# latk/hbetune.rs

Measured on AMD Instinct MI355X. Metric: GP fit+predict/sec (n=4096,d=8,f64), higher is better.
Workload: dtype f64; 1 GPU; M: rosenbrock d=8 n=4096 f64, Matern nu=5/2 x constant + white noise; fixed-work fit = 3 L-BFGS runs x 150 lml+gradient evaluations + K^-1, then predict mean+variance at m=1600; evals_per_fit=450, n_not_pd=0, m_candidates=1600, parallelism=replicas x1 (independent fits per GPU, no collective)

## Files before the change

### csrc/hbegp.cpp

```cpp
#include "../include/hbegp.h"

#include <hip/hip_runtime_api.h>

#include <algorithm>
#include <atomic>
#include <queue>
#include <cmath>
#include <cstdarg>
#include <cstdio>
#include <cstdlib>
#include <cstring>
#include <functional>
#include <limits>
#include <memory>
#include <mutex>
#include <numeric>
#include <string>
#include <thread>
#include <type_traits>
#include <vector>

#include "dag_plan.hpp"
#include "engine.hpp"
#include "lbfgsb.hpp"
#include "lbfgs_step.hpp"
#include "lockstep.hpp"


using namespace hbegp;

static thread_local std::string g_last_error = "";
static int fail(int code, const char* fmt, ...) {
  char buf[512];
  va_list ap;
  va_start(ap, fmt);
  vsnprintf(buf, sizeof(buf), fmt, ap);
  va_end(ap);
  g_last_error = buf;
  return code;
}
struct HipError {
// ... 549 lines not shown
  }
  off->assign(nwg + 1, 0);
  items->clear();
  for (int w = 0; w < nwg; ++w) {
    (*off)[w] = (int)items->size();
    items->insert(items->end(), per[w].begin(), per[w].end());
  }
  (*off)[nwg] = (int)items->size();
  *nwg_out = nwg;
  return true;
}

constexpr int DAG_MAX_VARIANTS = 4;
constexpr int DAG_CROWD_LEVELS = 3;
constexpr int DAG_CROWD_BUSY[DAG_CROWD_LEVELS] = {6, 12, 24};
constexpr int MAX_DEVS = 64;
struct DagPlanKey {
  int blocks, bk, small_h, nwg, lauum, rl, rl_group, rl_near, lauum_split, chain32, prog, big128;
  auto tie() const { return std::tie(blocks, bk, small_h, nwg, lauum, rl, rl_group, rl_near, lauum_split, chain32, prog, big128); }
  bool operator<(const DagPlanKey& o) const { return tie() < o.tie(); }
};
static std::atomic<int> g_dev_busy[MAX_DEVS];

template <typename T>
struct LooIn {
  int dev;
  hipStream_t s;
  int n, d, np, nu2;
  const T *X, *y, *alpha, *Xinv, *Kinv;
  const EvalParams* P;
};
template <typename T>
static int loo_tail(const LooIn<T>& in, T* mean, T* var, T* lpd, double* loo, double* grad);

template <typename T>
struct Slot {
  int dev = 0;
// ... 3 lines not shown
  T *W1 = nullptr, *W2 = nullptr, *Kinv[2] = {nullptr, nullptr}, *alpha[2] = {nullptr, nullptr};
  T* W3 = nullptr;
  T *ldiag = nullptr, *wbuf = nullptr;
  double *part_t = nullptr, *part_g = nullptr;
  EvalParams* dP = nullptr;
  EvalOut* dOut = nullptr;
  int* tickets = nullptr;
  unsigned long long* dag_trace = nullptr;
  int* dag_ctrl = nullptr;
  EvalParams* hP = nullptr;
  EvalOut* hOut = nullptr;
  void* small_slab = nullptr;
  size_t small_slab_bytes = 0;
  void* host_slab = nullptr;
  size_t host_slab_bytes = 0;
  hipGraphExec_t graph[DAG_MAX_VARIANTS + 1 + DAG_CROWD_LEVELS][2][4] = {};
  int best_idx = -1;
  double best_lml = -std::numeric_limits<double>::infinity();
  int best_run = 0, best_eval = 0;
  std::vector<double> best_theta;
  std::vector<double> best_params;
  int last_target = 0;
  int dag_variant = 1;
  int dag_part = 0;
  unsigned long long seq = 0;
  bool ctrl_cleared = false;
  bool published = false;
  long long expect_ns[4] = {0, 0, 0, 0};
};

struct ProblemBase {
// ... 19 lines not shown
  bool dag_lauum_ = false;
  bool dag_rl_ = false;
  double dag_gflop_lauum = 0;
  struct DagVariant {
    int nwg = 0;
    std::vector<DagTask*> tasks;
    std::vector<DagTask> host_tasks;
    int nwg_p1 = 0, ntasks_p1 = 0, nwg_kinv = 0, ntasks_kinv = 0;
    std::vector<DagTask*> tasks_p1, tasks_kinv;
    std::vector<DagTask> host_tasks_p1, host_tasks_kinv;
  };
  std::vector<DagVariant> dag_var;
  std::unique_ptr<std::atomic<int>[]> busy_slots_;
  int dag_ntasks = 0, dag_nwg = 0;
  int dag_nvar_ = 1, dag_ncrowd_ = 0;
  unsigned long long dag_wait_ticks_ = 200000000ull;
  size_t dag_ctrl_bytes = 0;
  int dag_ctrl_regions_ = 1;
  double dag_gflop = 0;
  bool adhoc_ = false;
  bool small_ = false;
  bool like_fit_ = false;
  bool lazy_ = false;
  std::function<std::shared_ptr<const DagPlan>(int, bool)> plan_for_;
  bool hostio_ = true;
  bool eval_published() const { return hostio_ && !small_; }
  int leaf_dbg_ = 0;

  struct Pooled { int dev; void* p; size_t bytes; };
  std::vector<Pooled> pooled_;
// ... 141 lines not shown
        if (!why.empty()) throw std::runtime_error("task queue of the factorisation is unsound: " + why);
      }
      if (dag_) {
        dag_ntasks = (int)plan.tasks.size();
        dag_nwg = std::min(dag_nwg, dag_ntasks);
        dag_gflop = plan.gflop;
        dag_gflop_lauum = plan.gflop_lauum;
        dag_ctrl_bytes = (sizeof(int) * (DAG_CTRL_WORDS + plan.totals.size()) + 15) / 16 * 16;
        dag_ctrl_regions_ = (lazy_ && dag_lauum_) ? 2 : 1;
        dag_wait_ticks_ = (unsigned long long)(std::max(2.0, 200.0 * plan.sim_us * 1e-6 * std::max(1, n_slots)) * 1e8);
        busy_slots_.reset(new std::atomic<int>[c->devs.size()]);
        for (size_t di = 0; di < c->devs.size(); ++di) busy_slots_[di].store(0);
        const bool adapt = env_int("HBEGP_DAG_ADAPT", 1) != 0 && forced <= 0;
        dag_nvar_ = nvar;
        dag_ncrowd_ = (adapt && n_slots > 1) ? DAG_CROWD_LEVELS : 0;
        dag_var.assign(nvar + 1 + dag_ncrowd_, DagVariant());
        for (int v = 1; v <= nvar + dag_ncrowd_; ++v) {
          DagVariant& var = dag_var[v];
          std::shared_ptr<const DagPlan> pv = cached;
          var.nwg = dag_nwg;
          if (v != nvar && adapt) {
            const int busy = v < nvar ? v : DAG_CROWD_BUSY[v - nvar - 1];
            var.nwg = std::min(share_of(busy), dag_ntasks);
            if (v > nvar) var.nwg = std::min(var.nwg, dag_nwg);
            pv = plan_for(var.nwg);
            if (pv->tasks.size() != plan.tasks.size()) { pv = cached; var.nwg = dag_nwg; }
          }
          var.host_tasks = pv->tasks;
          var.tasks.assign(c->devs.size(), nullptr);
          for (size_t di = 0; di < c->devs.size(); ++di) {
            HIPCHECK(hipSetDevice(c->devs[di]));
            var.tasks[di] = palloc<DagTask>(c->devs[di], pv->tasks.size());
            HIPCHECK(hipMemcpyAsync(var.tasks[di], var.host_tasks.data(), sizeof(DagTask) * var.host_tasks.size(), hipMemcpyHostToDevice, slots[di][0].stream));
          }
          if (lazy_ && dag_lauum_) {
            const int wg_p1 = lazy_wg(var.nwg, 1), wg_kinv = lazy_wg(var.nwg, 2);
            const std::shared_ptr<const DagPlan> p1 = plan_for_(wg_p1, false);
            const DagPlan kv = dag_plan_kinv_only(*pv);
            if (p1->tasks.empty() || kv.tasks.empty() || p1->totals.size() > plan.totals.size() || kv.totals.size() > plan.totals.size()) {
// ... 59 lines not shown
          HIPCHECK(hipMemcpyAsync(sc.d_items, items.data(), sizeof(unsigned) * items.size(), hipMemcpyHostToDevice, s.stream));
          HIPCHECK(hipStreamSynchronize(s.stream));
        }
        scheds[di].push_back(sc);
      };
      eval_gemms(s, s.Kinv[0], record, [](int) {}, [] {});
    }
  }
  ~Problem() override { release(); }

  void release() {
    for (size_t di = 0; di < slots.size(); ++di) {
      (void)hipSetDevice(ctx->devs[di]);
      for (auto& s : slots[di]) {
        if (s.stream) (void)hipStreamSynchronize(s.stream);
        for (int v = 0; v <= DAG_MAX_VARIANTS + DAG_CROWD_LEVELS; ++v)
          for (int a = 0; a < 2; ++a)
            for (int b = 0; b < 4; ++b)
              if (s.graph[v][a][b]) (void)hipGraphExecDestroy(s.graph[v][a][b]);
        const size_t nnb = sizeof(T) * (size_t)np * np;
        g_pool.put(s.dev, s.W1, nnb); g_pool.put(s.dev, s.W2, nnb); g_pool.put(s.dev, s.W3, nnb);
        for (int b = 0; b < 2; ++b) g_pool.put(s.dev, s.Kinv[b], nnb);
        g_pool.put(s.dev, s.small_slab, s.small_slab_bytes);
        g_host_pool.put(s.host_slab, s.host_slab_bytes);
        g_stream_pool.put(s.dev, s.stream);
      }
    }
    for (const Pooled& q : pooled_) g_pool.put(q.dev, q.p, q.bytes);
    pooled_.clear();
    slots.clear();
    scheds.clear();
// ... 272 lines not shown
    keep = base; keep.mi = keep.nj = q0; keep.c_lower = 1; keep.beta_one = 1;
    GemmOp& rect = g.op[g.nops++];
    rect = base; rect.ci0 = q0; rect.mi = nb - q0; rect.nj = q0; rect.klim = 4;
    GemmOp& tri = g.op[g.nops++];
    tri = base; tri.ci0 = tri.cj0 = q0; tri.mi = tri.nj = nb - q0; tri.c_lower = 1; tri.klim = 4;
    gemm_adhoc<T>(g, info, s.stream);
    CHECK_LAUNCHES();
    HIPCHECK(hipMemcpyAsync(s.hOut, s.dOut, sizeof(EvalOut), hipMemcpyDeviceToHost, s.stream));
    HIPCHECK(hipStreamSynchronize(s.stream));
    s.last_target = 0;
    if (s.hOut->info == 0 && !(s.hOut->done & 1)) throw HipError{hipErrorLaunchFailure, "extend: the evaluation kernels did not run", __LINE__};
    if (s.hOut->info == 0 && !std::isfinite(s.hOut->lml)) return HBEGP_NOT_PD;
    return s.hOut->info != 0 ? HBEGP_NOT_PD : HBEGP_OK;
  }

  int variant_now(size_t di) const {
    if (!dag_ || dag_var.size() < 2) return 1;
    const int nvar = dag_nvar_;
    const int busy = busy_slots_ ? busy_slots_[di].load(std::memory_order_relaxed) : 0;
    if (dag_ncrowd_ > 0) {
      const int dev = ctx->devs[di];
      const int total = dev < MAX_DEVS ? g_dev_busy[dev].load(std::memory_order_relaxed) : 0;
      if (total > std::max(busy, nvar)) {
        int l = 0;
        while (l + 1 < dag_ncrowd_ && DAG_CROWD_BUSY[l] < total) ++l;
        return nvar + 1 + l;
      }
    }
    return busy <= 0 ? nvar : std::min(busy, nvar);
  }
  int run_eval(size_t di, int si, int target, int mode, bool use_graph, double* lml, double* grad) {
    Slot<T>& s = slots[di][si];
    HIPCHECK(hipSetDevice(s.dev));
    static const bool graphs_on = env_int("HBEGP_NO_GRAPH", 0) == 0;
    const bool want_grad = mode == EVAL_FULL || mode == EVAL_GRAD_ONLY;
    if (mode == EVAL_GRAD_ONLY) {
      if (!lazy_ || !eval_published() || !grad) throw std::logic_error("run_eval: the gradient phase needs a lazily evaluated, published problem");
      reinterpret_cast<volatile unsigned long long*>(&s.hOut->seq)[0] = 0;
      std::atomic_thread_fence(std::memory_order_seq_cst);
    } else {
      s.dag_variant = variant_now(di);
      s.hP->seq = ++s.seq;
    }
    const auto t_launch = std::chrono::steady_clock::now();
    if (use_graph && graphs_on) {
      hipGraphExec_t& ge = s.graph[s.dag_variant][target][mode];
      if (!ge) {
        hipGraph_t gr = nullptr;
        HIPCHECK(hipStreamBeginCapture(s.stream, hipStreamCaptureModeThreadLocal));
        try {
          enqueue_eval(s, di, target, mode, nullptr);
        } catch (...) {
          (void)hipStreamEndCapture(s.stream, &gr);
          throw;
        }
        HIPCHECK(hipStreamEndCapture(s.stream, &gr));
// ... 1680 lines not shown
  if (!paths) return fail(HBEGP_EINVAL, "NULL paths handle");
  if (!starts || !lo || !hi || !x_best || !f_best) return fail(HBEGP_EINVAL, "starts/lo/hi/x_best/f_best is NULL");
  if (paths->is_f32 != (sizeof(T) == 4)) return fail(HBEGP_EINVAL, "paths handle holds %s data", paths->is_f32 ? "f32" : "f64");
  const int d = paths->model->d;
  if (d > LBFGS_MAXN) return fail(HBEGP_EINVAL, "d = %d exceeds the optimiser's %d variables", d, LBFGS_MAXN);
  for (int k = 0; k < d; ++k)
    if (!(lo[k] <= hi[k])) return fail(HBEGP_EINVAL, "lo[%d] > hi[%d] (%g > %g)", k, k, lo[k], hi[k]);
  for (size_t r = 0; r < (size_t)paths->S * R; ++r)
    for (int k = 0; k < d; ++k) {
      const double v = (double)starts[r * d + k];
      if (!(v >= lo[k] && v <= hi[k])) return fail(HBEGP_EINVAL, "start %zu lies outside the box (feature %d: %g)", r, k, v);
    }
  return HBEGP_OK;
}

struct LastFitStats { int n_evals, n_not_pd, n_lml_only; };
static thread_local LastFitStats g_last_fit_stats = {0, 0, 0};

static int read_fit_options(const hbegp_fit_options* in, hbegp_fit_options* out) {
  *out = hbegp_fit_options{};
  out->struct_size = sizeof(hbegp_fit_options);
  if (!in) return HBEGP_OK;
  if (in->struct_size < offsetof(hbegp_fit_options, maxeval) + sizeof(int) || in->struct_size > ((size_t)1 << 16))
    return fail(HBEGP_EINVAL, "hbegp_fit_options.struct_size = %zu: set it to sizeof(hbegp_fit_options) (HBEGP_FIT_OPTIONS_INIT)",
                in->struct_size);
  memcpy(out, in, std::min(in->struct_size, sizeof(*out)));
  return HBEGP_OK;
}

template <typename T>
static int do_extend(hbegp_ctx* ctx, const T* X, const T* y, int n, int d, double nu, const double* theta, const double* lo,
                     const double* hi, hbegp_model** model_out);

template <typename T>
static int do_fit(hbegp_ctx* ctx, const T* X, const T* y, int n, int d, double nu, const double* theta0, const double* lo,
                  const double* hi, const double* starts, int n_restarts, const hbegp_fit_options* opt_in,
                  double* theta_best, double* lml_best, hbegp_model** model_out, bool loo = false) {
  hbegp_fit_options opt{};
  g_last_fit_stats = {0, 0, 0};
  if (int e = read_fit_options(opt_in, &opt)) return e;
  if (opt.maxeval <= 0) opt.maxeval = 150;
  const int p = d + 2;
  const int nruns = 1 + std::max(0, n_restarts);
  const int ndev = (int)ctx->devs.size();
  const int max_conc = std::max(1, env_int("HBEGP_MAX_CONCURRENT", 3));
  std::vector<int> runs_on(ndev, 0);
  for (int r = 0; r < nruns; ++r) runs_on[r % ndev]++;
  int n_slots = 1;
  for (int di = 0; di < ndev; ++di) n_slots = std::max(n_slots, std::min(runs_on[di], max_conc));
  constexpr int SMALL_FIT_MAX_RUNS = 64;
  bool small_fit = !loo && round_up(n, NB) == NB && d <= SMALL_EVAL_MAXD && env_int("HBEGP_SMALL", 1) != 0 && env_int("HBEGP_SMALL_FIT", 1) != 0;
  for (int di = 0; di < ndev; ++di) small_fit = small_fit && runs_on[di] <= SMALL_FIT_MAX_RUNS;
  if (small_fit)
    for (int di = 0; di < ndev; ++di) n_slots = std::max(n_slots, runs_on[di]);
  static const int timing = env_int("HBEGP_TIMING", 0);
  const auto tf0 = std::chrono::steady_clock::now();
  SmallArrival arrival;
  if (small_fit) arrival.announce();
  static const int host_serial_max = env_int("HBEGP_SMALL_HOST_SERIAL", 16);
  struct SmallActive {
    bool on = false;
    int enter() { on = true; return g_small_active.fetch_add(1) + 1; }
    ~SmallActive() { if (on) g_small_active.fetch_sub(1); }
  } small_active;
  const bool host_serial = small_fit && small_active.enter() <= host_serial_max;
  std::unique_lock<std::mutex> host_lk(g_small_host_mu, std::defer_lock);
  if (host_serial) host_lk.lock();
  const auto th0 = std::chrono::steady_clock::now();
  double held_ms = 0;
  Problem<T> prob(ctx, X, y, n, d, nu, n_slots, false, true, !loo);
  const auto tf1 = std::chrono::steady_clock::now();
// ... 109 lines not shown
          } else {
            std::this_thread::sleep_for(microseconds(40));
            if (steady_clock::now() - last_query > milliseconds(20)) {
              last_query = steady_clock::now();
              const hipError_t e = hipStreamQuery(batches[di]->stream);
              if (e == hipSuccess) {
                if (*q == 1ull) break;
                throw HipError{hipErrorLaunchFailure, "small fit: the launch is over and a run never reported", __LINE__};
              }
              if (e != hipErrorNotReady) throw HipError{e, "hipStreamQuery (small-fit launch)", __LINE__};
            }
          }
        }
        std::atomic_thread_fence(std::memory_order_acquire);
      };
      for (int r = 0; r < nruns; ++r) wait_run(r, ws[r].di);
      runs_over = true;
      int total_evals = 0, total_not_pd = 0, trace_n = 0;
      for (int r = 0; r < nruns; ++r) {
        RunWs& w = ws[r];
        HIPCHECK(hipSetDevice(ctx->devs[w.di]));
        Slot<T>& s = prob.slots[w.di][w.si];
        hipStream_t st = prob.slots[w.di][0].stream;
        const SmallFitResult hr = hruns[r].res;
        total_evals += hr.n_evals;
        total_not_pd += hr.n_not_pd;
        s.best_idx = hr.best_idx;
        s.best_lml = hr.best_lml;
        s.best_run = r;
        s.best_eval = hr.best_eval;
        s.best_theta.assign(hr.best_theta, hr.best_theta + p);
        s.best_params.assign(hr.best_params, hr.best_params + p);
        s.last_target = hr.best_idx < 0 ? 0 : hr.best_idx;
        if (cap > 0 && trace_n < opt.trace_cap) {
          const int take = std::min(std::min(hr.n_evals, cap), opt.trace_cap - trace_n);
          if (opt.trace_theta) HIPCHECK(hipMemcpyAsync(opt.trace_theta + (size_t)trace_n * p, w.tr_theta, sizeof(double) * (size_t)take * p, hipMemcpyDeviceToHost, st));
          if (opt.trace_lml) HIPCHECK(hipMemcpyAsync(opt.trace_lml + trace_n, w.tr_lml, sizeof(double) * take, hipMemcpyDeviceToHost, st));
          if (opt.trace_grad) HIPCHECK(hipMemcpyAsync(opt.trace_grad + (size_t)trace_n * p, w.tr_grad, sizeof(double) * (size_t)take * p, hipMemcpyDeviceToHost, st));
          HIPCHECK(hipStreamSynchronize(st));
          if (opt.trace_run) for (int e = 0; e < take; ++e) opt.trace_run[trace_n + e] = r;
          trace_n += take;
        }
      }
      if (opt.trace_count) *opt.trace_count = trace_n;
      if (opt.n_evals) *opt.n_evals = total_evals;
      if (opt.n_not_pd) *opt.n_not_pd = total_not_pd;
      g_last_fit_stats = {total_evals, total_not_pd, 0};
      n_evals.store(total_evals);
    } catch (...) {
      for (int di = 0; di < ndev && di < (int)prob.slots.size(); ++di) {
        if (prob.slots[di].empty()) continue;
        (void)hipSetDevice(ctx->devs[di]);
        (void)hipStreamSynchronize(prob.slots[di][0].stream);
      }
      free_all();
      throw;
    }
    free_all();
  } else {
  if (prob.busy_slots_)
    for (int di = 0; di < ndev; ++di) prob.busy_slots_[di].store(std::min(runs_on[di], max_conc));
  auto worker = [&](int di, int si) {
    struct Leave {
      std::atomic<int>* busy;
      std::atomic<int>* dev_busy;
      ~Leave() {
        if (busy) busy->fetch_sub(1);
        if (dev_busy) dev_busy->fetch_sub(1);
      }
    } leave{prob.busy_slots_ ? &prob.busy_slots_[di] : nullptr, ctx->devs[di] < MAX_DEVS ? &g_dev_busy[ctx->devs[di]] : nullptr};
    if (leave.dev_busy) leave.dev_busy->fetch_add(1);
    try {
      HIPCHECK(hipSetDevice(ctx->devs[di]));
      Slot<T>& s = prob.slots[di][si];
      const int nslots_here = std::min(runs_on[di], max_conc);
      int local = 0;
      for (int r = di; r < nruns; r += ndev, ++local) {
        if (local % nslots_here != si) continue;
        std::vector<double> x(p);
        if (r == 0) for (int i = 0; i < p; ++i) x[i] = theta0[i];
        else for (int i = 0; i < p; ++i) x[i] = starts[(size_t)(r - 1) * p + i];
        int eval_idx = 0;
        auto obj = [&](const double* th, double* grad, const LbfgsState* ls) -> double {
          theta_to_params(th, lo, hi, d, s.hP);
          const int target = (s.best_idx < 0) ? 0 : 1 - s.best_idx;
          double lml;
          int st;
          if (ls) {
            st = prob.run_eval((size_t)di, si, target, Problem<T>::EVAL_LML_ONLY, true, &lml, nullptr);
            const bool new_best = st == HBEGP_OK && (s.best_idx < 0 || lml > s.best_lml);
            if (st == HBEGP_OK && (new_best || lbfgs_trial_accepted(*ls, -lml))) {
              st = prob.run_eval((size_t)di, si, target, Problem<T>::EVAL_GRAD_ONLY, true, nullptr, grad);
              if (st != HBEGP_OK) lml = -std::numeric_limits<double>::infinity();
            } else {
              for (int j = 0; j < p; ++j) grad[j] = 0.0;
              n_lml_only.fetch_add(1);
            }
          } else {
            st = prob.run_eval((size_t)di, si, target, !loo, true, &lml, loo ? nullptr : grad);
          }
          if (loo) {
            if (st == HBEGP_OK) st = prob.loo_on_slot((size_t)di, si, &lml, grad);
            else for (int j = 0; j < p; ++j) grad[j] = 0.0;
            if (st != HBEGP_OK && st != HBEGP_NOT_PD) throw std::runtime_error(g_last_error);
          }
          const int my_eval = eval_idx++;
          n_evals.fetch_add(1);
          if (st != HBEGP_OK) n_not_pd.fetch_add(1);
          if (opt.trace_cap > 0) {
            std::lock_guard<std::mutex> lk(trace_mu);
            if (trace_n < opt.trace_cap) {
              const int tI = trace_n++;
              if (opt.trace_theta) memcpy(opt.trace_theta + (size_t)tI * p, th, sizeof(double) * p);
              if (opt.trace_lml) opt.trace_lml[tI] = lml;
              if (opt.trace_grad) memcpy(opt.trace_grad + (size_t)tI * p, grad, sizeof(double) * p);
              if (opt.trace_run) opt.trace_run[tI] = r;
            }
          }
          if (st != HBEGP_OK) return std::numeric_limits<double>::infinity();
          if (s.best_idx < 0 || lml > s.best_lml) {
            s.best_idx = target;
// ... 6 lines not shown
          return -lml;
        };
        LbfgsOptions lo_opt;
        lo_opt.maxeval = opt.maxeval;
        lo_opt.fixed_work = opt.fixed_work != 0;
        if (opt.lbfgs_memory > 0) lo_opt.memory = opt.lbfgs_memory;
        static_assert(MAXP <= LBFGS_MAXN, "the GP's parameters fit the fixed-size optimiser state");
        std::vector<double> g(p);
        std::unique_ptr<LbfgsState> ls(new LbfgsState);
        lbfgs_begin(*ls, x.data(), lnlo.data(), lnhi.data(), p, lo_opt.maxeval, lo_opt.memory, lo_opt.pgtol, lo_opt.ftol, lo_opt.fixed_work);
        for (;;) {
          const bool trial = lazy && lbfgs_is_trial(*ls);
          const double f = obj(lbfgs_request(*ls), g.data(), trial ? ls.get() : nullptr);
          if (!lbfgs_advance(*ls, f, g.data())) break;
        }
      }
    } catch (const HipError& he) {
      hip_fail(he);
      std::lock_guard<std::mutex> lk(err_mu);
      err = g_last_error;
    } catch (const std::exception& e) {
      std::lock_guard<std::mutex> lk(err_mu);
      err = std::string("worker thread: ") + e.what();
    }
  };

  std::vector<std::thread> threads;
  try {
    for (int di = 0; di < ndev; ++di)
      for (int si = 0; si < std::min(runs_on[di], max_conc); ++si) threads.emplace_back(worker, di, si);
// ... 8 lines not shown
    std::stable_sort(order.begin(), order.end(), [&](int a, int b) { return opt.trace_run[a] < opt.trace_run[b]; });
    auto permute = [&](auto* arr, int width) {
      if (!arr) return;
      std::vector<typename std::remove_pointer<decltype(arr)>::type> tmp((size_t)trace_n * width);
      for (int i = 0; i < trace_n; ++i) memcpy(&tmp[(size_t)i * width], arr + (size_t)order[i] * width, sizeof(tmp[0]) * width);
      memcpy(arr, tmp.data(), sizeof(tmp[0]) * tmp.size());
    };
    permute(opt.trace_theta, p);
    permute(opt.trace_lml, 1);
    permute(opt.trace_grad, p);
    permute(opt.trace_run, 1);
  }
  if (opt.trace_count) *opt.trace_count = trace_n;
  if (opt.n_evals) *opt.n_evals = n_evals.load();
  if (opt.n_not_pd) *opt.n_not_pd = n_not_pd.load();
  g_last_fit_stats = {n_evals.load(), n_not_pd.load(), n_lml_only.load()};
  if (!err.empty()) return fail(HBEGP_EHIP, "%s", err.c_str());
  }

  int bdi = -1, bsi = -1;
  for (int di = 0; di < ndev; ++di)
    for (int si = 0; si < (int)prob.slots[di].size(); ++si) {
      const Slot<T>& s = prob.slots[di][si];
      if (s.best_idx < 0) continue;
      bool better = bdi < 0;
      if (!better) {
        const Slot<T>& b = prob.slots[bdi][bsi];
        better = s.best_lml > b.best_lml ||
                 (s.best_lml == b.best_lml && (s.best_run < b.best_run || (s.best_run == b.best_run && s.best_eval < b.best_eval)));
      }
      if (better) { bdi = di; bsi = si; }
    }
  if (bdi < 0) return fail(HBEGP_ALL_FAILED, "every evaluation of the fit failed (kernel matrix not positive definite)");
// ... 1209 lines not shown
void hbegp_model_retain(hbegp_model* model) {
  if (model) model->refs.fetch_add(1);
}
void hbegp_model_release(hbegp_model* model) {
  if (model && model->refs.fetch_sub(1) == 1) delete model;
}

int hbegp_last_fit_stats(hbegp_fit_stats* out) {
  if (!out || out->struct_size < offsetof(hbegp_fit_stats, n_evals) + sizeof(int) || out->struct_size > ((size_t)1 << 16))
    return fail(HBEGP_EINVAL, "hbegp_fit_stats.struct_size: set it to sizeof(hbegp_fit_stats) (HBEGP_FIT_STATS_INIT)");
  hbegp_fit_stats full{};
  full.struct_size = out->struct_size;
  full.n_evals = g_last_fit_stats.n_evals;
  full.n_not_pd = g_last_fit_stats.n_not_pd;
  full.n_lml_only = g_last_fit_stats.n_lml_only;
  memcpy(out, &full, std::min(out->struct_size, sizeof(full)));
  return HBEGP_OK;
}

static int lbfgs_replay_impl(int n, const double* x0, const double* lo, const double* hi, int maxeval, int memory, int fixed_work, int count,
                             const double* f, const double* g, double* requested, int* trial, int* accepted, int* took, int* n_requested) {
  LbfgsOptions o;
  std::unique_ptr<LbfgsState> st(new LbfgsState);
  lbfgs_begin(*st, x0, lo, hi, n, maxeval, memory > 0 ? memory : o.memory, o.pgtol, o.ftol, fixed_work != 0);
  memcpy(requested, lbfgs_request(*st), sizeof(double) * n);
  int produced = 1;
  for (int i = 0; i < count; ++i) {
    if (trial) {
      trial[i] = lbfgs_is_trial(*st) ? 1 : 0;
      accepted[i] = lbfgs_trial_accepted(*st, f[i]) ? 1 : 0;
// ... 8 lines not shown
    }
  }
  *n_requested = produced;
  return HBEGP_OK;
}

int hbegp_debug_lbfgs_decisions(int n, const double* x0, const double* lo, const double* hi, int maxeval, int memory, int fixed_work,
                                int count, const double* f, const double* g, double* requested, int* trial, int* accepted, int* took,
                                int* n_requested) {
  if (n < 1 || n > LBFGS_MAXN || count < 0 || !x0 || !lo || !hi || !requested || !n_requested || !trial || !accepted || !took ||
      (count > 0 && (!f || !g)))
    return fail(HBEGP_EINVAL, "bad argument");
  GUARD_BEGIN
  return lbfgs_replay_impl(n, x0, lo, hi, maxeval, memory, fixed_work, count, f, g, requested, trial, accepted, took, n_requested);
  GUARD_END
}

int hbegp_debug_dag_queues(int nblocks, int bk, int small_h, int nwg, int fine, int big128, int which, int* ntasks, int* tasks, int cap,
                           char* err, int errlen) {
  if (nblocks < 1 || (bk != 16 && bk != 32) || small_h < 0 || nwg < 0 || which < 0 || which > 2 || !ntasks) return fail(HBEGP_EINVAL, "bad argument");
  GUARD_BEGIN
  DagBuilder builder(bk, small_h, nwg, (fine & 1) != 0);
  builder.set_rl_progressive((fine & 16) != 0);
  builder.set_big128(big128 != 0, big128 >= 2);
  builder.set_rl(32, 1, (fine & 32) == 0, true);
  DagPlan plan = builder.build(0, nblocks, which != 1, (fine & 8) != 0);
  if (which == 2) plan = dag_plan_kinv_only(plan);
  const std::string why = plan.tasks.empty() ? std::string("no tasks") : dag_plan_validate(plan, nblocks);
  *ntasks = (int)plan.tasks.size();
  if (tasks)
// ... 73 lines not shown
```

### hbetune_rs_amd/_lib.py

```python
import ctypes as C
import os

import numpy as np

HERE = os.path.dirname(os.path.abspath(__file__))
LIB_PATH = os.environ.get("HBEGP_LIB") or os.path.join(HERE, "libhbegp.so")

OK, NOT_PD, ALL_FAILED = 0, 1, 2
EINVAL, EHIP, ENODEV, ENOMEM = -1, -2, -3, -4
PATHS_MAX_FEATURES, PATHS_MAX_PATHS = 16384, 1024
CEI_MAX_CONSTRAINTS = 8
MES_MAX_SAMPLES = 1024
EHVI_ND_MAX_BOXES = 1048576


class HbegpError(RuntimeError):
    def __init__(self, code, msg):
        super().__init__(f"hbegp error {code}: {msg}")
        self.code = code


class FitOptions(C.Structure):

    _fields_ = [
        ("struct_size", C.c_size_t),
        ("maxeval", C.c_int),
        ("fixed_work", C.c_int),
        ("lbfgs_memory", C.c_int),
# ... 2 lines not shown
        ("trace_lml", C.POINTER(C.c_double)),
        ("trace_grad", C.POINTER(C.c_double)),
        ("trace_run", C.POINTER(C.c_int)),
        ("trace_count", C.POINTER(C.c_int)),
        ("n_evals", C.POINTER(C.c_int)),
        ("n_not_pd", C.POINTER(C.c_int)),
    ]

    def __init__(self, *a, **k):
        super().__init__(*a, **k)
        self.struct_size = C.sizeof(FitOptions)


class FitStats(C.Structure):

    _fields_ = [("struct_size", C.c_size_t), ("n_evals", C.c_int), ("n_not_pd", C.c_int), ("n_lml_only", C.c_int)]

    def __init__(self, *a, **k):
        super().__init__(*a, **k)
        self.struct_size = C.sizeof(FitStats)


OBJECTIVE_FN = C.CFUNCTYPE(C.c_double, C.POINTER(C.c_double), C.POINTER(C.c_double), C.c_void_p)

_dp = C.POINTER(C.c_double)
_fp = C.POINTER(C.c_float)
_ip = C.POINTER(C.c_int)
_vp = C.c_void_p

SIGNATURES = {
    "hbegp_version": (C.c_int, []),
# ... 108 lines not shown
    "hbegp_debug_cei_phases": (C.c_int, [C.c_int, _dp]),
    "hbegp_debug_lcei_phases": (C.c_int, [C.c_int, _dp]),
    "hbegp_debug_mes_phases": (C.c_int, [C.c_int, _dp]),
    "hbegp_debug_pool_poisoned": (C.c_int, [C.POINTER(C.c_longlong), C.POINTER(C.c_longlong)]),
    "hbegp_model_info": (C.c_int, [_vp, _ip, _ip, _ip, _dp, _dp]),
    "hbegp_model_get_f64": (C.c_int, [_vp, _dp, _dp, _dp]),
    "hbegp_model_get_f32": (C.c_int, [_vp, _dp, _fp, _fp]),
    "hbegp_model_debug_params": (C.c_int, [_vp, _dp]),
    "hbegp_model_retain": (None, [_vp]),
    "hbegp_model_release": (None, [_vp]),
    "hbegp_debug_lbfgs_replay": (C.c_int, [C.c_int, _dp, _dp, _dp, C.c_int, C.c_int, C.c_int, C.c_int, _dp, _dp, _dp, _ip]),
    "hbegp_last_fit_stats": (C.c_int, [C.POINTER(FitStats)]),
    "hbegp_debug_lbfgs_decisions": (C.c_int, [C.c_int, _dp, _dp, _dp, C.c_int, C.c_int, C.c_int, C.c_int, _dp, _dp, _dp, _ip, _ip, _ip, _ip]),
    "hbegp_debug_dag_queues": (C.c_int, [C.c_int, C.c_int, C.c_int, C.c_int, C.c_int, C.c_int, C.c_int, _ip, _ip, C.c_int, C.c_char_p,
                                         C.c_int]),
    "hbegp_debug_dag_plan": (C.c_int, [C.c_int, C.c_int, C.c_int, C.c_int, C.c_int, _ip, _ip, _ip, _dp, _dp, _dp, C.c_char_p,
                                       C.c_int]),
    "hbegp_minimize_by_gradient": (C.c_double, [OBJECTIVE_FN, _vp, _dp, _dp, _dp, C.c_int, C.c_int]),
}

_lib = None


def load():
    global _lib
    if _lib is not None:
        return _lib
    if not os.path.exists(LIB_PATH):
        raise ImportError(
            f"{LIB_PATH} is missing: build it with `python -c 'import __graft_entry__ as g; g.build()'` or `make`. "
# ... 42 lines not shown
```

### hbetune_rs_amd/gpr.py

```python
import ctypes as C
import math

import numpy as np

from . import _lib
from ._lib import HbegpError, NOT_PD, ALL_FAILED


def _suffix(dtype):
    dt = np.dtype(dtype)
    if dt == np.float64:
        return "f64"
    if dt == np.float32:
        return "f32"
    raise TypeError(f"element type must be float64 or float32, got {dt}")


class Context:

    def __init__(self, n_devices=1, device_ids=None):
        lib = _lib.load()
        self._h = C.c_void_p()
        ids = None
        if device_ids is not None:
# ... 207 lines not shown
                opt.trace_grad = _lib.dptr(tr["grad"])
            opt.trace_run = tr["run"].ctypes.data_as(C.POINTER(C.c_int))
            opt.trace_count = C.pointer(tr["count"])
        handle = C.c_void_p()
        theta_best = np.zeros(p)
        lml_best = C.c_double()
        fit = getattr(lib, f"{symbol}_{sfx}")
        _lib.check(fit(ctx._h, _lib.aptr(x), _lib.aptr(y), n, d, float(nu), _lib.dptr(theta0), _lib.dptr(lo), _lib.dptr(hi),
                       _lib.dptr(starts_c), n_restarts, C.byref(opt), _lib.dptr(theta_best), C.byref(lml_best), C.byref(handle)))
        fk = FittedKernel(handle, dtype, n, d, nu)
        fk.x_train, fk.y_train = x, y
        fk.n_evals, fk.n_not_pd = n_evals.value, n_not_pd.value
        stats = _lib.FitStats()
        _lib.check(lib.hbegp_last_fit_stats(C.byref(stats)))
        fk.n_lml_only = stats.n_lml_only
        fk.theta_best = theta_best
        if symbol == "hbegp_fit_loo":
            fk.loo_best = lml_best.value
        if trace:
            k = tr["count"].value
            fk.trace = dict(theta=tr["theta"][:k], lml=tr["lml"][:k], run=tr["run"][:k])
            if trace != "lml":
                fk.trace["grad"] = tr["grad"][:k]
        return fk

    @staticmethod
    def extend(x_train, y_train, theta, lo=None, hi=None, nu=2.5, ctx=None):
        lib = _lib.load()
        ctx = ctx or default_context()
        dtype = np.dtype(x_train.dtype)
# ... 563 lines not shown
```

### include/hbegp.h

```cpp
#ifndef HBEGP_H
#define HBEGP_H

#include <stddef.h>

#ifdef __cplusplus
extern "C" {
#endif

#define HBEGP_VERSION 200

enum {
  HBEGP_OK = 0,
  HBEGP_NOT_PD = 1,
  HBEGP_ALL_FAILED = 2,
  HBEGP_EINVAL = -1,
  HBEGP_EHIP = -2,
  HBEGP_ENODEV = -3,
  HBEGP_ENOMEM = -4
};

typedef struct hbegp_ctx hbegp_ctx;
typedef struct hbegp_problem hbegp_problem;
typedef struct hbegp_model hbegp_model;

// ... 32 lines not shown
  size_t struct_size;
  int maxeval;
  int fixed_work;
  int lbfgs_memory;
  int trace_cap;
  double* trace_theta;
  double* trace_lml;
  double* trace_grad;
  int* trace_run;
  int* trace_count;
  int* n_evals;
  int* n_not_pd;
} hbegp_fit_options;
#define HBEGP_FIT_OPTIONS_INIT { sizeof(hbegp_fit_options) }

typedef struct hbegp_fit_stats {
  size_t struct_size;
  int n_evals;
  int n_not_pd;
  int n_lml_only;
} hbegp_fit_stats;
#define HBEGP_FIT_STATS_INIT { sizeof(hbegp_fit_stats) }
int hbegp_last_fit_stats(hbegp_fit_stats* out);

int hbegp_fit_f64(hbegp_ctx* ctx, const double* X, const double* y, int n, int d, double nu, const double* theta0,
                  const double* lo, const double* hi, const double* starts, int n_restarts,
                  const hbegp_fit_options* opt, double* theta_best, double* lml_best, hbegp_model** model);
int hbegp_fit_f32(hbegp_ctx* ctx, const float* X, const float* y, int n, int d, double nu, const double* theta0,
                  const double* lo, const double* hi, const double* starts, int n_restarts,
                  const hbegp_fit_options* opt, double* theta_best, double* lml_best, hbegp_model** model);

int hbegp_fit_loo_f64(hbegp_ctx* ctx, const double* X, const double* y, int n, int d, double nu, const double* theta0,
                      const double* lo, const double* hi, const double* starts, int n_restarts,
                      const hbegp_fit_options* opt, double* theta_best, double* loo_best, hbegp_model** model);
int hbegp_fit_loo_f32(hbegp_ctx* ctx, const float* X, const float* y, int n, int d, double nu, const double* theta0,
// ... 141 lines not shown

int hbegp_model_debug_params(hbegp_model* model, double* out);

int hbegp_debug_dag_plan(int nblocks, int bk, int small_h, int nwg, int fine, int* ntasks, int* ncounters, int* nleaf,
                         double* gflop, double* crit_us, double* sim_us, char* err, int errlen);

int hbegp_debug_lbfgs_replay(int n, const double* x0, const double* lo, const double* hi, int maxeval, int memory, int fixed_work,
                             int count, const double* f, const double* g, double* requested, int* n_requested);

int hbegp_debug_lbfgs_decisions(int n, const double* x0, const double* lo, const double* hi, int maxeval, int memory, int fixed_work,
                                int count, const double* f, const double* g, double* requested, int* trial, int* accepted, int* took,
                                int* n_requested);

int hbegp_debug_dag_queues(int nblocks, int bk, int small_h, int nwg, int fine, int big128, int which, int* ntasks, int* tasks, int cap,
                           char* err, int errlen);

int hbegp_debug_pool_poisoned(long long* blocks, long long* bytes);
int hbegp_debug_posterior_phases(int enable, double* phase_ms);
int hbegp_debug_batch_select_phases(int enable, double* phase_ms);
int hbegp_debug_kg_phases(int enable, double* phase_ms);
int hbegp_debug_nei_phases(int enable, double* phase_ms);
int hbegp_debug_ehvi_phases(int enable, double* phase_ms);
int hbegp_debug_ehvi_nd_phases(int enable, double* phase_ms);
int hbegp_debug_ehvi_boxes(const double* front, int P, int n_obj, const double* ref, int* thr_count, double* thr, int thr_cap,
                           int* n_boxes, int* boxes, int box_cap);
int hbegp_debug_cei_phases(int enable, double* phase_ms);
int hbegp_debug_lcei_phases(int enable, double* phase_ms);
int hbegp_debug_mes_phases(int enable, double* phase_ms);
int hbegp_debug_sens_phases(int enable, double* phase_ms);
int hbegp_debug_qei_phases(int enable, double* phase_ms);
// ... 25 lines not shown
```

Before: 1.931 fit+predict/s.

## Rebalance workgroups between concurrent L-BFGS runs by progress

Adds per-slot progress tracking so that, when several independent optimizer runs share one GPU, the slowest run gets a DAG factorisation variant with more workgroups and the others get fewer. The aim is to shrink the tail where the last run finishes alone on an underused device. Two extra graph variants are compiled per slot, and a hysteresis rule keeps shares from flapping. It also adds per-run stats reporting. The risk is extra plan and graph setup, plus contention if the shares are sized badly.

```diff
diff --git a/csrc/hbegp.cpp b/csrc/hbegp.cpp
--- a/csrc/hbegp.cpp
+++ b/csrc/hbegp.cpp
@@ -25,6 +25,7 @@
 #include "lbfgsb.hpp"
 #include "lbfgs_step.hpp"
 #include "lockstep.hpp"
+#include "slot_share.hpp"
 
 
 using namespace hbegp;
@@ -604,6 +605,7 @@
 constexpr int DAG_MAX_VARIANTS = 4;
 constexpr int DAG_CROWD_LEVELS = 3;
 constexpr int DAG_CROWD_BUSY[DAG_CROWD_LEVELS] = {6, 12, 24};
+constexpr int DAG_SHARE_VARIANTS = 2;
 constexpr int MAX_DEVS = 64;
 struct DagPlanKey {
   int blocks, bk, small_h, nwg, lauum, rl, rl_group, rl_near, lauum_split, chain32, prog, big128;
@@ -611,6 +613,7 @@
   bool operator<(const DagPlanKey& o) const { return tie() < o.tie(); }
 };
 static std::atomic<int> g_dev_busy[MAX_DEVS];
+static std::atomic<int> g_dev_fits[MAX_DEVS];
 
 template <typename T>
 struct LooIn {
@@ -644,7 +647,7 @@
   size_t small_slab_bytes = 0;
   void* host_slab = nullptr;
   size_t host_slab_bytes = 0;
-  hipGraphExec_t graph[DAG_MAX_VARIANTS + 1 + DAG_CROWD_LEVELS][2][4] = {};
+  hipGraphExec_t graph[DAG_MAX_VARIANTS + 1 + DAG_CROWD_LEVELS + DAG_SHARE_VARIANTS][2][4] = {};
   int best_idx = -1;
   double best_lml = -std::numeric_limits<double>::infinity();
   int best_run = 0, best_eval = 0;
@@ -694,6 +697,13 @@
   std::unique_ptr<std::atomic<int>[]> busy_slots_;
   int dag_ntasks = 0, dag_nwg = 0;
   int dag_nvar_ = 1, dag_ncrowd_ = 0;
+  int dag_nshare_ = 0;
+  int share_hyst_ = SLOT_SHARE_HYSTERESIS;
+  int slot_maxeval_ = 0;
+  std::vector<int> share_force_;
+  std::vector<char> balance_dev_;
+  std::unique_ptr<std::atomic<int>[]> slot_running_, slot_done_;
+  mutable std::atomic<int> not_alone_{0};
   unsigned long long dag_wait_ticks_ = 200000000ull;
   size_t dag_ctrl_bytes = 0;
   int dag_ctrl_regions_ = 1;
@@ -865,15 +875,43 @@
         const bool adapt = env_int("HBEGP_DAG_ADAPT", 1) != 0 && forced <= 0;
         dag_nvar_ = nvar;
         dag_ncrowd_ = (adapt && n_slots > 1) ? DAG_CROWD_LEVELS : 0;
-        dag_var.assign(nvar + 1 + dag_ncrowd_, DagVariant());
-        for (int v = 1; v <= nvar + dag_ncrowd_; ++v) {
+        int share_wg[DAG_SHARE_VARIANTS] = {slot_share_lead_wg(dag_nwg, n_slots, cus), slot_share_lag_wg(dag_nwg, n_slots, cus)};
+        if (const char* wgs = getenv("HBEGP_RUN_BALANCE_WG")) {
+          int a = 0, b = 0;
+          if (sscanf(wgs, "%d,%d", &a, &b) == 2 && a > 0 && b > 0) { share_wg[0] = std::min(a, cus); share_wg[1] = std::min(b, cus); }
+        }
+        const char* share_force = getenv("HBEGP_RUN_BALANCE_FORCE");
+        share_force_.clear();
+        if (share_force && *share_force) {
+          for (const char* q = share_force; *q;) {
+            const size_t len = strcspn(q, ",");
+            share_force_.push_back(strncmp(q, "lag", 3) == 0 ? SLOT_SHARE_LAG : (strncmp(q, "lead", 4) == 0 ? SLOT_SHARE_LEAD : SLOT_SHARE_EVEN));
+            q += len;
+            if (*q == ',') ++q;
+          }
+          share_force_.resize(n_slots, SLOT_SHARE_EVEN);
+        }
+        share_hyst_ = std::max(0, env_int("HBEGP_RUN_BALANCE_HYST", SLOT_SHARE_HYSTERESIS));
+        dag_nshare_ = (adapt && n_slots > 1 && (env_int("HBEGP_RUN_BALANCE", np / NB >= SLOT_SHARE_MIN_BLOCKS ? 1 : 0) != 0 || !share_force_.empty())) ? DAG_SHARE_VARIANTS : 0;
+        if (dag_nshare_) {
+          balance_dev_.assign(c->devs.size(), 0);
+          slot_running_.reset(new std::atomic<int>[c->devs.size() * n_slots]);
+          slot_done_.reset(new std::atomic<int>[c->devs.size() * n_slots]);
+          for (size_t i = 0; i < c->devs.size() * n_slots; ++i) { slot_running_[i].store(0); slot_done_[i].store(0); }
+        }
+        dag_var.assign(nvar + 1 + dag_ncrowd_ + dag_nshare_, DagVariant());
+        for (int v = 1; v <= nvar + dag_ncrowd_ + dag_nshare_; ++v) {
           DagVariant& var = dag_var[v];
           std::shared_ptr<const DagPlan> pv = cached;
           var.nwg = dag_nwg;
           if (v != nvar && adapt) {
-            const int busy = v < nvar ? v : DAG_CROWD_BUSY[v - nvar - 1];
-            var.nwg = std::min(share_of(busy), dag_ntasks);
-            if (v > nvar) var.nwg = std::min(var.nwg, dag_nwg);
+            if (v > nvar + dag_ncrowd_) {
+              var.nwg = std::min(share_wg[v - nvar - dag_ncrowd_ - 1], dag_ntasks);
+            } else {
+              const int busy = v < nvar ? v : DAG_CROWD_BUSY[v - nvar - 1];
+              var.nwg = std::min(share_of(busy), dag_ntasks);
+              if (v > nvar) var.nwg = std::min(var.nwg, dag_nwg);
+            }
             pv = plan_for(var.nwg);
             if (pv->tasks.size() != plan.tasks.size()) { pv = cached; var.nwg = dag_nwg; }
           }
@@ -963,7 +1001,7 @@
       (void)hipSetDevice(ctx->devs[di]);
       for (auto& s : slots[di]) {
         if (s.stream) (void)hipStreamSynchronize(s.stream);
-        for (int v = 0; v <= DAG_MAX_VARIANTS + DAG_CROWD_LEVELS; ++v)
+        for (int v = 0; v <= DAG_MAX_VARIANTS + DAG_CROWD_LEVELS + DAG_SHARE_VARIANTS; ++v)
           for (int a = 0; a < 2; ++a)
             for (int b = 0; b < 4; ++b)
               if (s.graph[v][a][b]) (void)hipGraphExecDestroy(s.graph[v][a][b]);
@@ -1266,7 +1304,7 @@
     return s.hOut->info != 0 ? HBEGP_NOT_PD : HBEGP_OK;
   }
 
-  int variant_now(size_t di) const {
+  int variant_now(size_t di, int si = -1) const {
     if (!dag_ || dag_var.size() < 2) return 1;
     const int nvar = dag_nvar_;
     const int busy = busy_slots_ ? busy_slots_[di].load(std::memory_order_relaxed) : 0;
@@ -1279,9 +1317,31 @@
         return nvar + 1 + l;
       }
     }
+    if (si >= 0 && dag_nshare_ > 0 && ctx->devs[di] < MAX_DEVS && g_dev_fits[ctx->devs[di]].load(std::memory_order_relaxed) > 1)
+      not_alone_.store(1, std::memory_order_relaxed);
+    if (si >= 0 && dag_nshare_ > 0 && busy == n_slots && n_slots >= 2 && n_slots <= SLOT_SHARE_MAX_SLOTS && balance_dev_[di] &&
+        !not_alone_.load(std::memory_order_relaxed)) {
+      int share[SLOT_SHARE_MAX_SLOTS];
+      if (!share_force_.empty()) {
+        for (int i = 0; i < n_slots; ++i) share[i] = share_force_[i];
+      } else {
+        int running[SLOT_SHARE_MAX_SLOTS], done[SLOT_SHARE_MAX_SLOTS], cap[SLOT_SHARE_MAX_SLOTS];
+        for (int i = 0; i < n_slots; ++i) {
+          running[i] = slot_running_[di * n_slots + i].load(std::memory_order_relaxed);
+          done[i] = slot_done_[di * n_slots + i].load(std::memory_order_relaxed);
+          cap[i] = slot_maxeval_;
+        }
+        slot_shares(n_slots, running, done, cap, share_hyst_, share);
+      }
+      if (share[si] != SLOT_SHARE_EVEN) return nvar + dag_ncrowd_ + (share[si] == SLOT_SHARE_LEAD ? 1 : 2);
+    }
     return busy <= 0 ? nvar : std::min(busy, nvar);
   }
-  int run_eval(size_t di, int si, int target, int mode, bool use_graph, double* lml, double* grad) {
+  int share_of_variant(int v) const {
+    if (!dag_ || dag_nshare_ <= 0 || v <= dag_nvar_ + dag_ncrowd_) return SLOT_SHARE_EVEN;
+    return v == dag_nvar_ + dag_ncrowd_ + 1 ? SLOT_SHARE_LEAD : SLOT_SHARE_LAG;
+  }
+  int run_eval(size_t di, int si, int target, int mode, bool use_graph, double* lml, double* grad, bool in_run = false) {
     Slot<T>& s = slots[di][si];
     HIPCHECK(hipSetDevice(s.dev));
     static const bool graphs_on = env_int("HBEGP_NO_GRAPH", 0) == 0;
@@ -1291,7 +1351,7 @@
       reinterpret_cast<volatile unsigned long long*>(&s.hOut->seq)[0] = 0;
       std::atomic_thread_fence(std::memory_order_seq_cst);
     } else {
-      s.dag_variant = variant_now(di);
+      s.dag_variant = variant_now(di, in_run ? si : -1);
       s.hP->seq = ++s.seq;
     }
     const auto t_launch = std::chrono::steady_clock::now();
@@ -3002,8 +3062,12 @@
   return HBEGP_OK;
 }
 
-struct LastFitStats { int n_evals, n_not_pd, n_lml_only; };
-static thread_local LastFitStats g_last_fit_stats = {0, 0, 0};
+struct RunStats { double end_ms = 0; int fused = 0, lml_only = 0, phase2 = 0, lead = 0, lag = 0; };
+struct LastFitStats {
+  int n_evals = 0, n_not_pd = 0, n_lml_only = 0, n_runs = 0;
+  RunStats run[HBEGP_STATS_MAX_RUNS];
+};
+static thread_local LastFitStats g_last_fit_stats;
 
 static int read_fit_options(const hbegp_fit_options* in, hbegp_fit_options* out) {
   *out = hbegp_fit_options{};
@@ -3025,7 +3089,7 @@
                   const double* hi, const double* starts, int n_restarts, const hbegp_fit_options* opt_in,
                   double* theta_best, double* lml_best, hbegp_model** model_out, bool loo = false) {
   hbegp_fit_options opt{};
-  g_last_fit_stats = {0, 0, 0};
+  g_last_fit_stats = LastFitStats{};
   if (int e = read_fit_options(opt_in, &opt)) return e;
   if (opt.maxeval <= 0) opt.maxeval = 150;
   const int p = d + 2;
@@ -3043,6 +3107,13 @@
     for (int di = 0; di < ndev; ++di) n_slots = std::max(n_slots, runs_on[di]);
   static const int timing = env_int("HBEGP_TIMING", 0);
   const auto tf0 = std::chrono::steady_clock::now();
+  auto since_start_ms = [tf0] { return std::chrono::duration<double, std::milli>(std::chrono::steady_clock::now() - tf0).count(); };
+  std::vector<RunStats> run_stats(nruns);
+  struct FitsInFlight {
+    const hbegp_ctx* c;
+    explicit FitsInFlight(const hbegp_ctx* cc) : c(cc) { for (int dev : c->devs) if (dev < MAX_DEVS) g_dev_fits[dev].fetch_add(1); }
+    ~FitsInFlight() { for (int dev : c->devs) if (dev < MAX_DEVS) g_dev_fits[dev].fetch_sub(1); }
+  } fits_in_flight(ctx);
   SmallArrival arrival;
   if (small_fit) arrival.announce();
   static const int host_serial_max = env_int("HBEGP_SMALL_HOST_SERIAL", 16);
@@ -3182,7 +3253,11 @@
         }
         std::atomic_thread_fence(std::memory_order_acquire);
       };
-      for (int r = 0; r < nruns; ++r) wait_run(r, ws[r].di);
+      for (int r = 0; r < nruns; ++r) {
+        wait_run(r, ws[r].di);
+        run_stats[r].end_ms = since_start_ms();
+        run_stats[r].fused = hruns[r].res.n_evals;
+      }
       runs_over = true;
       int total_evals = 0, total_not_pd = 0, trace_n = 0;
       for (int r = 0; r < nruns; ++r) {
@@ -3213,7 +3288,9 @@
       if (opt.trace_count) *opt.trace_count = trace_n;
       if (opt.n_evals) *opt.n_evals = total_evals;
       if (opt.n_not_pd) *opt.n_not_pd = total_not_pd;
-      g_last_fit_stats = {total_evals, total_not_pd, 0};
+      g_last_fit_stats.n_evals = total_evals;
+      g_last_fit_stats.n_not_pd = total_not_pd;
+      g_last_fit_stats.n_lml_only = 0;
       n_evals.store(total_evals);
     } catch (...) {
       for (int di = 0; di < ndev && di < (int)prob.slots.size(); ++di) {
@@ -3228,6 +3305,10 @@
   } else {
   if (prob.busy_slots_)
     for (int di = 0; di < ndev; ++di) prob.busy_slots_[di].store(std::min(runs_on[di], max_conc));
+  if (prob.dag_nshare_ > 0) {
+    prob.slot_maxeval_ = opt.maxeval;
+    for (int di = 0; di < ndev; ++di) prob.balance_dev_[di] = runs_on[di] <= max_conc && runs_on[di] == prob.n_slots;
+  }
   auto worker = [&](int di, int si) {
     struct Leave {
       std::atomic<int>* busy;
@@ -3249,30 +3330,43 @@
         if (r == 0) for (int i = 0; i < p; ++i) x[i] = theta0[i];
         else for (int i = 0; i < p; ++i) x[i] = starts[(size_t)(r - 1) * p + i];
         int eval_idx = 0;
+        RunStats& rs = run_stats[r];
+        std::atomic<int>* progress = prob.dag_nshare_ > 0 ? &prob.slot_done_[(size_t)di * prob.n_slots + si] : nullptr;
+        if (progress) {
+          progress->store(0, std::memory_order_relaxed);
+          prob.slot_running_[(size_t)di * prob.n_slots + si].store(1, std::memory_order_relaxed);
+        }
         auto obj = [&](const double* th, double* grad, const LbfgsState* ls) -> double {
           theta_to_params(th, lo, hi, d, s.hP);
           const int target = (s.best_idx < 0) ? 0 : 1 - s.best_idx;
           double lml;
           int st;
           if (ls) {
-            st = prob.run_eval((size_t)di, si, target, Problem<T>::EVAL_LML_ONLY, true, &lml, nullptr);
+            st = prob.run_eval((size_t)di, si, target, Problem<T>::EVAL_LML_ONLY, true, &lml, nullptr, true);
             const bool new_best = st == HBEGP_OK && (s.best_idx < 0 || lml > s.best_lml);
             if (st == HBEGP_OK && (new_best || lbfgs_trial_accepted(*ls, -lml))) {
               st = prob.run_eval((size_t)di, si, target, Problem<T>::EVAL_GRAD_ONLY, true, nullptr, grad);
               if (st != HBEGP_OK) lml = -std::numeric_limits<double>::infinity();
+              rs.phase2++;
             } else {
               for (int j = 0; j < p; ++j) grad[j] = 0.0;
               n_lml_only.fetch_add(1);
+              rs.lml_only++;
             }
           } else {
-            st = prob.run_eval((size_t)di, si, target, !loo, true, &lml, loo ? nullptr : grad);
+            st = prob.run_eval((size_t)di, si, target, !loo, true, &lml, loo ? nullptr : grad, true);
+            rs.fused++;
           }
+          const int share = prob.share_of_variant(s.dag_variant);
+          if (share == SLOT_SHARE_LEAD) rs.lead++;
+          if (share == SLOT_SHARE_LAG) rs.lag++;
           if (loo) {
             if (st == HBEGP_OK) st = prob.loo_on_slot((size_t)di, si, &lml, grad);
             else for (int j = 0; j < p; ++j) grad[j] = 0.0;
             if (st != HBEGP_OK && st != HBEGP_NOT_PD) throw std::runtime_error(g_last_error);
           }
           const int my_eval = eval_idx++;
+          if (progress) progress->store(eval_idx, std::memory_order_relaxed);
           n_evals.fetch_add(1);
           if (st != HBEGP_OK) n_not_pd.fetch_add(1);
           if (opt.trace_cap > 0) {
@@ -3309,6 +3403,8 @@
           const double f = obj(lbfgs_request(*ls), g.data(), trial ? ls.get() : nullptr);
           if (!lbfgs_advance(*ls, f, g.data())) break;
         }
+        rs.end_ms = since_start_ms();
+        if (progress) prob.slot_running_[(size_t)di * prob.n_slots + si].store(0, std::memory_order_relaxed);
       }
     } catch (const HipError& he) {
       hip_fail(he);
@@ -3347,9 +3443,18 @@
   if (opt.trace_count) *opt.trace_count = trace_n;
   if (opt.n_evals) *opt.n_evals = n_evals.load();
   if (opt.n_not_pd) *opt.n_not_pd = n_not_pd.load();
-  g_last_fit_stats = {n_evals.load(), n_not_pd.load(), n_lml_only.load()};
+  g_last_fit_stats.n_evals = n_evals.load();
+  g_last_fit_stats.n_not_pd = n_not_pd.load();
+  g_last_fit_stats.n_lml_only = n_lml_only.load();
   if (!err.empty()) return fail(HBEGP_EHIP, "%s", err.c_str());
   }
+
+  g_last_fit_stats.n_runs = std::min(nruns, (int)HBEGP_STATS_MAX_RUNS);
+  for (int r = 0; r < g_last_fit_stats.n_runs; ++r) g_last_fit_stats.run[r] = run_stats[r];
+  if (timing)
+    for (int r = 0; r < nruns; ++r)
+      fprintf(stderr, "fit: run %d ended at %.2f ms: %d fused, %d lml-only, %d two-phase evaluations; %d with a lead share, %d with a lag share\n", r,
+              run_stats[r].end_ms, run_stats[r].fused, run_stats[r].lml_only, run_stats[r].phase2, run_stats[r].lead, run_stats[r].lag);
 
   int bdi = -1, bsi = -1;
   for (int di = 0; di < ndev; ++di)
@@ -4589,6 +4694,13 @@
   full.n_evals = g_last_fit_stats.n_evals;
   full.n_not_pd = g_last_fit_stats.n_not_pd;
   full.n_lml_only = g_last_fit_stats.n_lml_only;
+  full.n_runs = g_last_fit_stats.n_runs;
+  for (int r = 0; r < full.n_runs; ++r) {
+    const RunStats& rs = g_last_fit_stats.run[r];
+    full.run_end_ms[r] = rs.end_ms;
+    full.run_fused[r] = rs.fused; full.run_lml_only[r] = rs.lml_only; full.run_phase2[r] = rs.phase2;
+    full.run_lead[r] = rs.lead; full.run_lag[r] = rs.lag;
+  }
   memcpy(out, &full, std::min(out->struct_size, sizeof(full)));
   return HBEGP_OK;
 }
@@ -4627,6 +4739,19 @@
   GUARD_BEGIN
   return lbfgs_replay_impl(n, x0, lo, hi, maxeval, memory, fixed_work, count, f, g, requested, trial, accepted, took, n_requested);
   GUARD_END
+}
+
+int hbegp_debug_slot_shares(int n_slots, const int* running, const int* done, const int* maxeval, int hysteresis, int* share, int even_wg,
+                            int cus, int* lead_wg, int* lag_wg) {
+  if (n_slots < 1 || !running || !done || !maxeval || !share) return fail(HBEGP_EINVAL, "bad argument");
+  slot_shares(n_slots, running, done, maxeval, hysteresis < 0 ? SLOT_SHARE_HYSTERESIS : hysteresis, share);
+  if (lead_wg) *lead_wg = slot_share_lead_wg(even_wg, n_slots, cus);
+  if (lag_wg) *lag_wg = slot_share_lag_wg(even_wg, n_slots, cus);
+  return HBEGP_OK;
+}
+
+int hbegp_debug_fits_in_flight(int device_id) {
+  return device_id >= 0 && device_id < MAX_DEVS ? g_dev_fits[device_id].load() : 0;
 }
 
 int hbegp_debug_dag_queues(int nblocks, int bk, int small_h, int nwg, int fine, int big128, int which, int* ntasks, int* tasks, int cap,
diff --git a/csrc/slot_share.hpp b/csrc/slot_share.hpp
--- /dev/null
+++ b/csrc/slot_share.hpp
@@ -0,0 +1,31 @@
+#pragma once
+#include <algorithm>
+
+enum SlotShare { SLOT_SHARE_EVEN = 0, SLOT_SHARE_LEAD = 1, SLOT_SHARE_LAG = 2 };
+
+constexpr int SLOT_SHARE_HYSTERESIS = 2;
+constexpr int SLOT_SHARE_STEP_WG = 16;
+constexpr int SLOT_SHARE_MAX_SLOTS = 8;
+constexpr int SLOT_SHARE_MIN_BLOCKS = 32;
+
+inline int slot_share_lead_wg(int even_wg, int , int cus) { return std::max(8, std::min(cus, even_wg - SLOT_SHARE_STEP_WG)); }
+inline int slot_share_lag_wg(int even_wg, int n_slots, int cus) {
+  return std::max(8, std::min(cus, even_wg + SLOT_SHARE_STEP_WG * std::max(1, n_slots - 1)));
+}
+
+inline void slot_shares(int n_slots, const int* running, const int* done, const int* maxeval, int hysteresis, int* share) {
+  int last = -1, n_running = 0;
+  for (int i = 0; i < n_slots; ++i) {
+    share[i] = SLOT_SHARE_EVEN;
+    if (!running[i] || done[i] >= maxeval[i]) continue;
+    ++n_running;
+    if (last < 0 || done[i] < done[last]) last = i;
+  }
+  if (n_running < 2) return;
+  for (int i = 0; i < n_slots; ++i) {
+    if (i == last || !running[i] || done[i] >= maxeval[i]) continue;
+    if ((long long)done[i] - done[last] <= hysteresis) return;
+  }
+  for (int i = 0; i < n_slots; ++i)
+    if (running[i] && done[i] < maxeval[i]) share[i] = i == last ? SLOT_SHARE_LAG : SLOT_SHARE_LEAD;
+}
diff --git a/hbetune_rs_amd/_lib.py b/hbetune_rs_amd/_lib.py
--- a/hbetune_rs_amd/_lib.py
+++ b/hbetune_rs_amd/_lib.py
@@ -12,6 +12,7 @@
 CEI_MAX_CONSTRAINTS = 8
 MES_MAX_SAMPLES = 1024
 EHVI_ND_MAX_BOXES = 1048576
+STATS_MAX_RUNS = 16
 
 
 class HbegpError(RuntimeError):
@@ -44,7 +45,10 @@
 
 class FitStats(C.Structure):
 
-    _fields_ = [("struct_size", C.c_size_t), ("n_evals", C.c_int), ("n_not_pd", C.c_int), ("n_lml_only", C.c_int)]
+    _fields_ = [("struct_size", C.c_size_t), ("n_evals", C.c_int), ("n_not_pd", C.c_int), ("n_lml_only", C.c_int), ("n_runs", C.c_int),
+                ("run_end_ms", C.c_double * STATS_MAX_RUNS), ("run_fused", C.c_int * STATS_MAX_RUNS),
+                ("run_lml_only", C.c_int * STATS_MAX_RUNS), ("run_phase2", C.c_int * STATS_MAX_RUNS),
+                ("run_lead", C.c_int * STATS_MAX_RUNS), ("run_lag", C.c_int * STATS_MAX_RUNS)]
 
     def __init__(self, *a, **k):
         super().__init__(*a, **k)
@@ -183,6 +187,8 @@
     "hbegp_debug_lbfgs_decisions": (C.c_int, [C.c_int, _dp, _dp, _dp, C.c_int, C.c_int, C.c_int, C.c_int, _dp, _dp, _dp, _ip, _ip, _ip, _ip]),
     "hbegp_debug_dag_queues": (C.c_int, [C.c_int, C.c_int, C.c_int, C.c_int, C.c_int, C.c_int, C.c_int, _ip, _ip, C.c_int, C.c_char_p,
                                          C.c_int]),
+    "hbegp_debug_slot_shares": (C.c_int, [C.c_int, _ip, _ip, _ip, C.c_int, _ip, C.c_int, C.c_int, _ip, _ip]),
+    "hbegp_debug_fits_in_flight": (C.c_int, [C.c_int]),
     "hbegp_debug_dag_plan": (C.c_int, [C.c_int, C.c_int, C.c_int, C.c_int, C.c_int, _ip, _ip, _ip, _dp, _dp, _dp, C.c_char_p,
                                        C.c_int]),
     "hbegp_minimize_by_gradient": (C.c_double, [OBJECTIVE_FN, _vp, _dp, _dp, _dp, C.c_int, C.c_int]),
diff --git a/hbetune_rs_amd/gpr.py b/hbetune_rs_amd/gpr.py
--- a/hbetune_rs_amd/gpr.py
+++ b/hbetune_rs_amd/gpr.py
@@ -245,6 +245,10 @@
         stats = _lib.FitStats()
         _lib.check(lib.hbegp_last_fit_stats(C.byref(stats)))
         fk.n_lml_only = stats.n_lml_only
+        k = stats.n_runs
+        fk.run_end_ms = np.array(stats.run_end_ms[:k], dtype=np.float64)
+        fk.run_counts = {name: np.array(getattr(stats, "run_" + name)[:k], dtype=np.int64)
+                         for name in ("fused", "lml_only", "phase2", "lead", "lag")}
         fk.theta_best = theta_best
         if symbol == "hbegp_fit_loo":
             fk.loo_best = lml_best.value
diff --git a/include/hbegp.h b/include/hbegp.h
--- a/include/hbegp.h
+++ b/include/hbegp.h
@@ -70,11 +70,19 @@
 } hbegp_fit_options;
 #define HBEGP_FIT_OPTIONS_INIT { sizeof(hbegp_fit_options) }
 
+#define HBEGP_STATS_MAX_RUNS 16
 typedef struct hbegp_fit_stats {
   size_t struct_size;
   int n_evals;
   int n_not_pd;
   int n_lml_only;
+  int n_runs;
+  double run_end_ms[HBEGP_STATS_MAX_RUNS];
+  int run_fused[HBEGP_STATS_MAX_RUNS];
+  int run_lml_only[HBEGP_STATS_MAX_RUNS];
+  int run_phase2[HBEGP_STATS_MAX_RUNS];
+  int run_lead[HBEGP_STATS_MAX_RUNS];
+  int run_lag[HBEGP_STATS_MAX_RUNS];
 } hbegp_fit_stats;
 #define HBEGP_FIT_STATS_INIT { sizeof(hbegp_fit_stats) }
 int hbegp_last_fit_stats(hbegp_fit_stats* out);
@@ -246,6 +254,10 @@
 
 int hbegp_debug_dag_queues(int nblocks, int bk, int small_h, int nwg, int fine, int big128, int which, int* ntasks, int* tasks, int cap,
                            char* err, int errlen);
+
+int hbegp_debug_slot_shares(int n_slots, const int* running, const int* done, const int* maxeval, int hysteresis, int* share, int even_wg,
+                            int cus, int* lead_wg, int* lag_wg);
+int hbegp_debug_fits_in_flight(int device_id);
 
 int hbegp_debug_pool_poisoned(long long* blocks, long long* bytes);
 int hbegp_debug_posterior_phases(int enable, double* phase_ms);
```

Result: faster. 1.979 fit+predict/s, median of 6 (+2.5%).
